# Vasilispapg/CVML-GoalNet

Measured on AMD Instinct MI355X. Metric: training clips/sec at batch 64, 16-frame 224² clips; logit MAE vs CPU ref, higher is better.
Workload: dtype f32; 1 GPU; AVM train step (forward + broadcast-MSE + backward + fused Adam), 64 clips x 16 frames = 1024 frames of 3x224x224 + 30x30 MFCC per GPU; dropout live (device masks), BatchNorm train mode; frames_per_gpu=1024, h=224, w=224, parallelism=dp1, ddp_semantics=local BN + local MSE per rank, gradient mean (standard DDP), params=1286754369

## Files before the change

### cvml_goalnet_amd/csrc/gemm_f32.hip

```cpp
#include <stdlib.h>

#include "gemm_common.h"
#include "skinny.h"

using namespace goalnet;

namespace {

constexpr int BM = 128, BN = 128, BK = 32;
constexpr int LDR = 128;
constexpr int OP_FLOATS = BM * BK;

__device__ __forceinline__ int kc_off(int row, int chunk) { return row * BK + ((chunk ^ ((row >> 1) & 7)) << 2); }

__device__ __forceinline__ float4 f4zero() { return make_float4(0.f, 0.f, 0.f, 0.f); }
__device__ __forceinline__ float4 f4fma(float4 v, float4 s, float4 t) {
    return make_float4(fmaf(v.x, s.x, t.x), fmaf(v.y, s.y, t.y), fmaf(v.z, s.z, t.z), fmaf(v.w, s.w, t.w));
}

typedef unsigned int u32x4 __attribute__((ext_vector_type(4)));
constexpr unsigned OOB = 0xFFFFFF00u;

__device__ __forceinline__ float4 f4sel(bool v, float4 a) { return v ? a : f4zero(); }

// ... 329 lines not shown
    for (int j = blockIdx.x * blockDim.x + threadIdx.x; j < Mpad / 4; j += gridDim.x * blockDim.x) {
        const int kt = j >> 3, k0 = j & 7;
        uint32_t word = 0;
#pragma unroll
        for (int i = 0; i < 4; ++i) {
            const int m = kt * 32 + k0 + 8 * i;
            const int w = m % W, h = (m / W) % H;
            const uint32_t c = m < M ? (uint32_t)((h == 0 ? 1 : 0) | (h == H - 1 ? 2 : 0) | (w == 0 ? 4 : 0) | (w == W - 1 ? 8 : 0)) : 0xFu;
            word |= c << (8 * i);
        }
        codes4[j] = word;
    }
}

__global__ __launch_bounds__(256) void wgrad_border_sums_kernel(const float* __restrict__ dy, double* __restrict__ parts,
                                                               int H, int W, int Cout) {
    const int n = blockIdx.x;
    const float* f = dy + (int64_t)n * H * W * Cout;
    double* out = parts + (int64_t)n * 8 * Cout;
    for (int c = threadIdx.x; c < Cout; c += blockDim.x) {
        double r0 = 0, r1 = 0, c0 = 0, c1 = 0;
        for (int w = 0; w < W; ++w) { r0 += (double)f[(int64_t)w * Cout + c]; r1 += (double)f[((int64_t)(H - 1) * W + w) * Cout + c]; }
        for (int h = 0; h < H; ++h) { c0 += (double)f[(int64_t)h * W * Cout + c]; c1 += (double)f[((int64_t)h * W + W - 1) * Cout + c]; }
        out[0 * Cout + c] = r0; out[1 * Cout + c] = r1; out[2 * Cout + c] = c0; out[3 * Cout + c] = c1;
        out[4 * Cout + c] = (double)f[c];
        out[5 * Cout + c] = (double)f[(int64_t)(W - 1) * Cout + c];
        out[6 * Cout + c] = (double)f[(int64_t)(H - 1) * W * Cout + c];
        out[7 * Cout + c] = (double)f[((int64_t)(H - 1) * W + W - 1) * Cout + c];
    }
}

__device__ __forceinline__ float border_u_of(const double* v, int tap) {
    const int kh = tap / 3, kw = tap - 3 * kh;
    double r = (kh == 0 ? v[0] : 0.0) + (kh == 2 ? v[1] : 0.0) + (kw == 0 ? v[2] : 0.0) + (kw == 2 ? v[3] : 0.0);
    if (kh == 0 && kw == 0) r -= v[4];
    if (kh == 0 && kw == 2) r -= v[5];
    if (kh == 2 && kw == 0) r -= v[6];
    if (kh == 2 && kw == 2) r -= v[7];
    return (float)r;
}

__global__ __launch_bounds__(256) void wgrad_border_u_kernel(const double* __restrict__ parts, int N, int Cout, float* __restrict__ u) {
    __shared__ double s[32][8];
    const int cl = threadIdx.x & 31, j = threadIdx.x >> 5;
    const int c = blockIdx.x * 32 + cl;
    double a0 = 0, a1 = 0, a2 = 0, a3 = 0;
    if (c < Cout) {
        const double* q = parts + (int64_t)j * Cout + c;
        int n = 0;
        for (; n + 3 < N; n += 4) {
            a0 += q[(int64_t)n * 8 * Cout]; a1 += q[(int64_t)(n + 1) * 8 * Cout];
            a2 += q[(int64_t)(n + 2) * 8 * Cout]; a3 += q[(int64_t)(n + 3) * 8 * Cout];
        }
        for (; n < N; ++n) a0 += q[(int64_t)n * 8 * Cout];
    }
    s[cl][j] = (a0 + a1) + (a2 + a3);
    __syncthreads();
    for (int t = threadIdx.x; t < 32 * 9; t += 256) {
        const int cc = t / 9, tap = t - 9 * cc;
        if (blockIdx.x * 32 + cc < Cout) u[(int64_t)(blockIdx.x * 32 + cc) * 9 + tap] = border_u_of(s[cc], tap);
    }
}

template <bool KC>
__device__ __forceinline__ void store_tile(float* l, const float4 (&r)[4], int tid) {
    if (KC) {
        const int c4 = (tid & 7) * 4, row = tid >> 3;
#pragma unroll
        for (int i = 0; i < 4; ++i) *reinterpret_cast<float4*>(&l[kc_off(row + 32 * i, c4 >> 2)]) = r[i];
    } else {
        const int r4 = (tid & 31) * 4, k = tid >> 5;
#pragma unroll
        for (int i = 0; i < 4; ++i) *reinterpret_cast<float4*>(&l[(k + 8 * i) * LDR + r4]) = r[i];
    }
}

template <bool KC>
__device__ __forceinline__ void read_group(const float* l, int strip, int s, int r, int h, float (&f)[2][4]) {
    if (KC) {
#pragma unroll
        for (int q = 0; q < 2; ++q) {
            const float4 t = *reinterpret_cast<const float4*>(&l[kc_off(strip + q * 32 + r, 2 * s + h)]);
            f[q][0] = t.x; f[q][1] = t.y; f[q][2] = t.z; f[q][3] = t.w;
        }
    } else {
#pragma unroll
        for (int j = 0; j < 4; ++j) {
            const float2 t = *reinterpret_cast<const float2*>(&l[(8 * s + 4 * h + j) * LDR + strip + 2 * r]);
            f[0][j] = t.x; f[1][j] = t.y;
        }
    }
}

template <bool AKC, bool BKC>
__device__ __forceinline__ void compute_tile(const float* la, const float* lb, f32x16 (&acc)[2][2],
                                             int wm, int wn, int r, int h) {
#pragma unroll
    for (int s = 0; s < 4; ++s) {
        float a[2][4], b[2][4];
        read_group<AKC>(la, wm * 64, s, r, h, a);
        read_group<BKC>(lb, wn * 64, s, r, h, b);
#pragma unroll
        for (int j = 0; j < 4; ++j) {
#pragma unroll
            for (int fm = 0; fm < 2; ++fm)
#pragma unroll
                for (int fn = 0; fn < 2; ++fn)
                    acc[fm][fn] = __builtin_amdgcn_mfma_f32_32x32x2f32(a[fm][j], b[fn][j], acc[fm][fn], 0, 0, 0);
        }
    }
}

template <bool BKC>
__device__ __forceinline__ void compute_tile_strip(const float* ls, const float* lb, f32x16 (&acc)[2][2],
                                                   const unsigned (&ab)[2], int wn, int r, int h) {
    static_assert(BKC, "K-contiguous B image");
    const unsigned bb = (unsigned)kc_off(wn * 64 + r, h) * 4;
#pragma unroll
    for (int s = 0; s < 4; ++s) {
        float a[2][4], b[2][4];
#pragma unroll
        for (int q = 0; q < 2; ++q) {
            const float4 t = *reinterpret_cast<const float4*>(reinterpret_cast<const char*>(ls) + (ab[q] ^ (unsigned)(s << 5)));
            a[q][0] = t.x; a[q][1] = t.y; a[q][2] = t.z; a[q][3] = t.w;
            const float4 u = *reinterpret_cast<const float4*>(reinterpret_cast<const char*>(lb) + ((bb ^ (unsigned)(s << 5)) + q * 32 * BK * 4));
            b[q][0] = u.x; b[q][1] = u.y; b[q][2] = u.z; b[q][3] = u.w;
        }
#pragma unroll
        for (int j = 0; j < 4; ++j) {
#pragma unroll
            for (int fm = 0; fm < 2; ++fm)
#pragma unroll
                for (int fn = 0; fn < 2; ++fn)
                    acc[fm][fn] = __builtin_amdgcn_mfma_f32_32x32x2f32(a[fm][j], b[fn][j], acc[fm][fn], 0, 0, 0);
        }
    }
}

template <class AL, class BL>
__device__ __forceinline__ void conv_strip_loop(AL& al, BL& bl, float* ls, float* lb, f32x16 (&acc)[2][2], int ktiles,
                                                int tid, int wn, int r, int h) {
    float4 rs[STRIP_LOADS], rb[4];
    const int nchunks = ktiles / 9;
    if (tid < 8) *reinterpret_cast<float4*>(&ls[STRIP_ROWS * BK + tid * 4]) = f4zero();
    al.begin(0);
#pragma unroll
    for (int i = 0; i < STRIP_LOADS; ++i) rs[i] = al.load(0, i);
    bl.issue(0, rb);
    al.store(ls, rs, tid);
    bl.finish(rb);
    store_tile<BL::KC>(lb, rb, tid);
    __syncthreads();
    for (int chunk = 0; chunk < nchunks; ++chunk) {
        const bool next = chunk + 1 < nchunks;
#pragma unroll
        for (int tap = 0; tap < 9; ++tap) {
            const bool more = tap < 8 || next;
            if (more) bl.issue(chunk * 9 + tap + 1, rb);
            if (next) rs[tap] = al.load(chunk + 1, tap);
            unsigned ab[2];
            al.frag_base(tap, ab);
            compute_tile_strip<BL::KC>(ls, lb, acc, ab, wn, r, h);
            __syncthreads();
            if (more) {
                bl.finish(rb);
                store_tile<BL::KC>(lb, rb, tid);
            }
            if (tap == 8 && next) {
                al.begin(chunk + 1);
                al.store(ls, rs, tid);
            }
            __syncthreads();
        }
    }
}

__device__ __forceinline__ void compute_tile_n64(const float* la, const float* lb, f32x16 (&acc)[2], int wave, int r, int h) {
#pragma unroll
    for (int s = 0; s < 4; ++s) {
        const float4 ta = *reinterpret_cast<const float4*>(&la[kc_off(wave * 32 + r, 2 * s + h)]);
        const float4 tb0 = *reinterpret_cast<const float4*>(&lb[kc_off(r, 2 * s + h)]);
        const float4 tb1 = *reinterpret_cast<const float4*>(&lb[kc_off(32 + r, 2 * s + h)]);
        const float a[4] = {ta.x, ta.y, ta.z, ta.w}, b0[4] = {tb0.x, tb0.y, tb0.z, tb0.w}, b1[4] = {tb1.x, tb1.y, tb1.z, tb1.w};
#pragma unroll
        for (int j = 0; j < 4; ++j) {
            acc[0] = __builtin_amdgcn_mfma_f32_32x32x2f32(a[j], b0[j], acc[0], 0, 0, 0);
            acc[1] = __builtin_amdgcn_mfma_f32_32x32x2f32(a[j], b1[j], acc[1], 0, 0, 0);
        }
    }
}

__device__ __forceinline__ void store_acc_n64(const EpiP& ep, const f32x16 (&acc)[2], int tm, int tn, int split, int wave, int r, int h) {
    float* outp = ep.slab_stride > 0 ? (ep.slabs ? ep.slabs : ep.out) + (int64_t)split * ep.slab_stride : ep.out;
    const int mode = ep.slab_stride > 0 ? EPI_RAW : ep.mode;
    const int64_t ld = (ep.slab_stride > 0 && ep.slabs) ? (int64_t)ep.cols : ep.ld;
#pragma unroll
    for (int fn = 0; fn < 2; ++fn) {
        const int col = tn * 64 + fn * 32 + r;
        const bool colok = col < ep.cols;
        const int64_t row0 = (int64_t)tm * BM + wave * 32 + 4 * h;
        const float bv = (mode == EPI_BIAS_RELU && ep.bias) ? ep.bias[colok ? col : 0] : 0.f;
        const float lo = (mode == EPI_BIAS_RELU && ep.relu) ? 0.f : -INFINITY;
#pragma unroll
        for (int e = 0; e < 16; ++e) {
            const int64_t row = row0 + (e & 3) + 8 * (e >> 2);
            if (!(colok && row < ep.rows)) continue;
            const float v = acc[fn][e];
            if (mode == EPI_RAW) outp[row * ld + col] = v;
            else if (mode == EPI_BIAS_RELU) outp[row * ld + col] = fmaxf(v + bv, lo);
            else outp[row * ld + col] = epi_apply(ep, v, row, col);
        }
    }
}

template <class AL, class BL, bool N64 = false, int STAGES = 2>
__global__ __launch_bounds__(256, STAGES == 1 ? (N64 ? 4 : AL::ONE_STAGE_BLOCKS) : 2) void gemm_f32_kernel(typename AL::P ap, typename BL::P bp, EpiP ep,
                                                          int tiles_m, int tiles_n, int m_fast,
                                                          int ktiles, int ktiles_per_split, int xcd_splits) {
    const int tid = threadIdx.x;
    int tm, tn, split;
    if (xcd_splits > 0) {
        const int tiles = tiles_m * tiles_n;
        const int xcd = blockIdx.x & 7, j = blockIdx.x >> 3;
        int t;
        if (tiles > 64 && tiles <= 128) {
            const int gs = (xcd_splits + 7) / 8, rest = tiles - 64, nA = gs * 64;
            int q;
            if (j < nA) { q = j >> 6; t = j & 63; }
            else { const int i = j - nA; q = i / rest; t = 64 + (i - q * rest); }
            split = q * 8 + xcd;
        } else {
            split = (j / tiles) * 8 + xcd;
            t = j - (j / tiles) * tiles;
        }
        if (split >= xcd_splits) return;
        if (m_fast) { tm = t % tiles_m; tn = t / tiles_m; } else { tn = t % tiles_n; tm = t / tiles_n; }
    } else {
        tile_of_block(tiles_m, tiles_n, m_fast, tm, tn);
        split = blockIdx.y;
    }
    const int kt0 = split * ktiles_per_split;
    const int kt1 = min(ktiles, kt0 + ktiles_per_split);

    static_assert(!N64 || (AL::KC && BL::KC), "the 128 x 64 tile reads K-contiguous LDS images");
    AL al(ap, tm * BM, tid);
    BL bl(bp, tn * (N64 ? 64 : BN), tid);

    const int lane = tid & 63, wave = tid >> 6;
    const int wm = wave >> 1, wn = wave & 1;
    const int r = lane & 31, h = lane >> 5;

    f32x16 acc[2][2];
#pragma unroll
    for (int i = 0; i < 2; ++i)
#pragma unroll
        for (int j = 0; j < 2; ++j)
#pragma unroll
            for (int e = 0; e < 16; ++e) acc[i][j][e] = 0.f;

    if constexpr (AL::STRIP) {
        static_assert(!N64 && STAGES == 1 && BL::KC, "the strip form: 128 x 128 tile, one B stage");
        __shared__ __attribute__((aligned(16))) float lstrip[STRIP_FLOATS];
        __shared__ __attribute__((aligned(16))) float lbs[OP_FLOATS];
        conv_strip_loop(al, bl, lstrip, lbs, acc, kt1 - kt0, tid, wn, r, h);
    } else {
        __shared__ __attribute__((aligned(16))) float lds[STAGES][2][OP_FLOATS];
        float4 ra[4], rb[4];
        if (kt0 < kt1) {
            al.issue(kt0, ra);
            bl.issue(kt0, rb);
            al.finish(ra);
            bl.finish(rb);
            store_tile<AL::KC>(lds[0][0], ra, tid);
            store_tile<BL::KC>(lds[0][1], rb, tid);
        }
        __syncthreads();
        for (int kt = kt0; kt < kt1; ++kt) {
            const int cur = STAGES == 1 ? 0 : (kt - kt0) & 1;
            const bool more = kt + 1 < kt1;
            if (more) {
                al.issue(kt + 1, ra);
                bl.issue(kt + 1, rb);
            }
            if constexpr (N64) compute_tile_n64(lds[cur][0], lds[cur][1], acc[0], wave, r, h);
            else compute_tile<AL::KC, BL::KC>(lds[cur][0], lds[cur][1], acc, wm, wn, r, h);
            if constexpr (STAGES == 1) __syncthreads();
            if (more) {
                al.finish(ra);
                bl.finish(rb);
                store_tile<AL::KC>(lds[STAGES == 1 ? 0 : cur ^ 1][0], ra, tid);
                store_tile<BL::KC>(lds[STAGES == 1 ? 0 : cur ^ 1][1], rb, tid);
            }
            __syncthreads();
        }
    }
    if constexpr (N64) store_acc_n64(ep, acc[0], tm, tn, split, wave, r, h);
    else store_acc<!AL::KC, !BL::KC>(ep, acc, tm, tn, split, wm, wn, r, h);
    if (ep.tile_ctr) {
        const int nsp = (ktiles + ktiles_per_split - 1) / ktiles_per_split;
        fused_splitk_reduce<N64 ? 64 : BN>(ep, tm, tn, tm * tiles_n + tn, nsp, tid);
    }
}

__global__ __launch_bounds__(256) void splitk_reduce_kernel(const float* slabs, int nsplit, int64_t slab_stride, EpiP ep) {
    const int c4n = ep.cols >> 2;
    const int64_t total = (int64_t)ep.rows * c4n;
    for (int64_t i = (int64_t)blockIdx.x * blockDim.x + threadIdx.x; i < total; i += (int64_t)gridDim.x * blockDim.x) {
        const int64_t row = i / c4n;
        const int col = (int)(i - row * c4n) * 4;
        const float* s = slabs + row * ep.cols + col;
        float4 a = *reinterpret_cast<const float4*>(s);
        for (int k = 1; k < nsplit; ++k) {
            const float4 b = *reinterpret_cast<const float4*>(s + (int64_t)k * slab_stride);
            a.x += b.x; a.y += b.y; a.z += b.z; a.w += b.w;
        }
        if (ep.oscale) { const int k = *ep.oscale; a.x = ldexpf(a.x, k); a.y = ldexpf(a.y, k); a.z = ldexpf(a.z, k); a.w = ldexpf(a.w, k); }
        if (ep.corr_u) {
            const int tap = col / ep.corr_C, ci = col - tap * ep.corr_C;
            const float u = ep.corr_u[row * 9 + tap];
            const float4 shv = *reinterpret_cast<const float4*>(ep.corr_sh + ci);
            a.x = fmaf(-shv.x, u, a.x); a.y = fmaf(-shv.y, u, a.y); a.z = fmaf(-shv.z, u, a.z); a.w = fmaf(-shv.w, u, a.w);
        }
        float* o = ep.out + row * ep.ld + col;
        o[0] = epi_apply(ep, a.x, row, col);
        o[1] = epi_apply(ep, a.y, row, col + 1);
        o[2] = epi_apply(ep, a.z, row, col + 2);
        o[3] = epi_apply(ep, a.w, row, col + 3);
    }
}

__global__ __launch_bounds__(256) void splitk_reduce_wide_kernel(const float* slabs, int nsplit, int64_t slab_stride, EpiP ep) {
    const int c4n = ep.cols >> 2;
    const int64_t total = (int64_t)ep.rows * c4n;
    const int g = threadIdx.x & 15;
    const int64_t step = (int64_t)gridDim.x * 16;
    const int64_t rounds = (total + step - 1) / step;
    int64_t i = (int64_t)blockIdx.x * 16 + (threadIdx.x >> 4);
    for (int64_t r = 0; r < rounds; ++r, i += step) {
        const bool ok = i < total;
        const int64_t ic = ok ? i : 0;
        const int64_t row = ic / c4n;
        const int col = (int)(ic - row * c4n) * 4;
        const float* s = slabs + row * ep.cols + col;
        float4 a = make_float4(0.f, 0.f, 0.f, 0.f);
        for (int k = g; k < nsplit; k += 16) {
            const float4 b = *reinterpret_cast<const float4*>(s + (int64_t)k * slab_stride);
            a.x += b.x; a.y += b.y; a.z += b.z; a.w += b.w;
        }
        a.x = row16_sum(a.x); a.y = row16_sum(a.y); a.z = row16_sum(a.z); a.w = row16_sum(a.w);
        if (ep.oscale) { const int k = *ep.oscale; a.x = ldexpf(a.x, k); a.y = ldexpf(a.y, k); a.z = ldexpf(a.z, k); a.w = ldexpf(a.w, k); }
        if (ep.corr_u) {
            const int tap = col / ep.corr_C, ci = col - tap * ep.corr_C;
            const float u = ep.corr_u[row * 9 + tap];
            const float4 shv = *reinterpret_cast<const float4*>(ep.corr_sh + ci);
            a.x = fmaf(-shv.x, u, a.x); a.y = fmaf(-shv.y, u, a.y); a.z = fmaf(-shv.z, u, a.z); a.w = fmaf(-shv.w, u, a.w);
        }
        if (ok && g == 0) {
            float* o = ep.out + row * ep.ld + col;
            o[0] = epi_apply(ep, a.x, row, col);
            o[1] = epi_apply(ep, a.y, row, col + 1);
            o[2] = epi_apply(ep, a.z, row, col + 2);
            o[3] = epi_apply(ep, a.w, row, col + 3);
        }
    }
}

template <class AL, class BL, bool N64 = false>
int launch_gemm(const char* name, const typename AL::P& ap, const typename BL::P& bp, const EpiP& ep,
                int64_t M, int64_t N, int ktiles, int nsplit, int m_fast, hipStream_t st) {
    const int64_t tiles_m = (M + BM - 1) / BM, tiles_n = (N + (N64 ? 64 : BN) - 1) / (N64 ? 64 : BN);
    GN_REQUIRE(tiles_m * tiles_n < (1ll << 31), GOALNET_E_SHAPE, "%s: too many tiles", name);
    GN_REQUIRE(nsplit >= 1 && nsplit <= 65535, GOALNET_E_SHAPE, "%s: bad split count %d", name, nsplit);
    const int kps = (ktiles + nsplit - 1) / nsplit;
    GN_REQUIRE(!ep.tile_ctr || (ktiles + kps - 1) / kps == nsplit, GOALNET_E_SHAPE, "%s: fused split-K needs every split non-empty", name);
    const bool xcd_local = nsplit >= 8 && tiles_m * tiles_n <= 256 && tiles_m * tiles_n * ((nsplit + 7) / 8 * 8) < (1ll << 31);
    dim3 grid((unsigned)(tiles_m * tiles_n), (unsigned)nsplit, 1);
    if (xcd_local) grid = dim3((unsigned)(tiles_m * tiles_n * ((nsplit + 7) / 8 * 8)), 1, 1);
    static const int force_stages = getenv("GOALNET_F32_STAGES") ? atoi(getenv("GOALNET_F32_STAGES")) : 0;
    const bool one_stage = AL::STRIP || force_stages == 1 || (force_stages != 2 && AL::ONE_STAGE);
    if (one_stage) {
        hipLaunchKernelGGL((gemm_f32_kernel<AL, BL, N64, 1>), grid, dim3(256), 0, st, ap, bp, ep, (int)tiles_m, (int)tiles_n,
                           m_fast, ktiles, kps, xcd_local ? nsplit : 0);
        GN_LAUNCH_CHECK(name);
        return 0;
    }
    if constexpr (!AL::STRIP) {
        hipLaunchKernelGGL((gemm_f32_kernel<AL, BL, N64>), grid, dim3(256), 0, st, ap, bp, ep, (int)tiles_m, (int)tiles_n,
                           m_fast, ktiles, kps, xcd_local ? nsplit : 0);
        GN_LAUNCH_CHECK(name);
    }
    return 0;
}

}

namespace goalnet {
int launch_splitk_reduce(const char* name, const float* slabs, int nsplit, int64_t slab_stride, const EpiP& ep, hipStream_t st) {
    const int64_t total = (int64_t)ep.rows * (ep.cols >> 2);
    int64_t blocks = (total + 255) / 256;
    if (blocks > 4096) blocks = 4096;
    if (blocks < 1) blocks = 1;
    if (total < 65536 && nsplit >= 32) {
        int64_t wb = (total + 15) / 16;
        if (wb > 4096) wb = 4096;
        hipLaunchKernelGGL(splitk_reduce_wide_kernel, dim3((unsigned)wb), dim3(256), 0, st, slabs, nsplit, slab_stride, ep);
        GN_LAUNCH_CHECK(name);
        return 0;
    }
    hipLaunchKernelGGL(splitk_reduce_kernel, dim3((unsigned)blocks), dim3(256), 0, st, slabs, nsplit, slab_stride, ep);
    GN_LAUNCH_CHECK(name);
    return 0;
}

int pick_splits(int64_t tiles, int ktiles) {
    if (ktiles < 8 || (ktiles < 64 && tiles >= 128)) return 1;
    int64_t s = ((ktiles < 64 ? 256 : 1024) + tiles - 1) / tiles;
    const int64_t smax = ktiles < 64 ? ktiles / 4 : (ktiles / 8 > 1 ? ktiles / 8 : 1);
    if (s > smax) s = smax;
    if (s < 1) s = 1;
    const int kps = (int)((ktiles + s - 1) / s);
    return (ktiles + kps - 1) / kps;
}

}

extern "C" {

static int conv_splits_f32(int64_t M, int Cin, int Cout) {
    return conv_fwd_splits(((M + BM - 1) / BM) * ((Cout + BN - 1) / BN), 9 * Cin / BK);
}

constexpr bool CONV_STRIP_FWD = true;
constexpr bool CONV_STRIP_DGRAD = true;
static bool conv_strip_f32(int W, int nsplit, bool narrow, bool affine) {
    const char* e = getenv("GOALNET_F32_CONV_STRIP");
    if (e && e[0] == '0') return false;
    return nsplit == 1 && !narrow && W <= CONV_STRIP_MAX_W && (affine ? CONV_STRIP_FWD : CONV_STRIP_DGRAD);
}

size_t goalnet_conv3x3_fwd_ws_bytes(int N, int H, int W, int Cin, int Cout) {
    if (N <= 0 || H <= 0 || W <= 0 || Cin <= 0 || Cout <= 0) return 0;
    const int64_t M = (int64_t)N * H * W;
    const int s = conv_splits_f32(M, Cin, Cout);
    return s > 1 ? (size_t)s * (size_t)M * (size_t)Cout * sizeof(float) : 0;
}

int goalnet_conv3x3_fwd(const float* x, const float* scale, const float* shift, const float* w,
                        const float* bias, int relu, float* y, int N, int H, int W, int Cin, int Cout,
                        void* ws, size_t ws_bytes, int* tile_ctr, int n_ctr, void* stream) {
    GN_REQUIRE(x && w && y, GOALNET_E_NULL, "conv3x3_fwd: null pointer");
    GN_REQUIRE((scale == nullptr) == (shift == nullptr), GOALNET_E_NULL, "conv3x3_fwd: scale/shift must both be set or both NULL");
    GN_REQUIRE(N > 0 && H > 0 && W > 0 && Cin > 0 && Cout > 0, GOALNET_E_SHAPE, "conv3x3_fwd: non-positive dim");
    GN_REQUIRE(Cin % BK == 0, GOALNET_E_SHAPE, "conv3x3_fwd: Cin=%d must be a multiple of %d", Cin, BK);
    GN_REQUIRE(Cout % 4 == 0, GOALNET_E_SHAPE, "conv3x3_fwd: Cout=%d must be a multiple of 4", Cout);
    GN_REQUIRE(aligned16(x) && aligned16(w) && aligned16(y) && aligned16(scale) && aligned16(shift),
               GOALNET_E_ALIGN, "conv3x3_fwd: pointers must be 16-byte aligned");
    const int64_t M = (int64_t)N * H * W;
    GN_REQUIRE(M < (1ll << 31) - 256, GOALNET_E_SHAPE, "conv3x3_fwd: N*H*W too large");
    hipStream_t st = (hipStream_t)stream;
    KCLoader<false>::P bp{w, (int64_t)9 * Cin, Cout, nullptr, nullptr, 1, Cin};
    const EpiP efinal{EPI_BIAS_RELU, y, Cout, (int)M, Cout, bias, relu, nullptr, 0, nullptr, 0, 0};
    EpiP ep = efinal;
    const int ktiles = 9 * Cin / BK;
    int nsplit = ws ? conv_splits_f32(M, Cin, Cout) : 1;
    if (nsplit > 1) {
        GN_REQUIRE(aligned16(ws) && ws_bytes >= goalnet_conv3x3_fwd_ws_bytes(N, H, W, Cin, Cout), GOALNET_E_WORKSPACE,
                   "conv3x3_fwd: workspace too small or misaligned");
        ep = EpiP{EPI_RAW, (float*)ws, Cout, (int)M, Cout, nullptr, 0, nullptr, 0, nullptr, 0, M * Cout};
    }
    const bool narrow = Cout <= 64 && !getenv("GOALNET_F32_N64_OFF");
    const bool fused = nsplit > 1 && tile_ctr && (int64_t)n_ctr >= ((M + BM - 1) / BM) * ((Cout + (narrow ? 64 : BN) - 1) / (narrow ? 64 : BN));
    if (fused) {
        ep = efinal;
        ep.slabs = (float*)ws; ep.slab_stride = M * Cout; ep.tile_ctr = tile_ctr;
    }
    const bool strip = conv_strip_f32(W, nsplit, narrow, scale != nullptr);
    int rc;
    if (strip && scale) {
        ConvAStripLoader<true>::P ap{x, H, W, Cin, M, scale, shift};
        rc = launch_gemm<ConvAStripLoader<true>, KCLoader<false>>("conv3x3_fwd", ap, bp, ep, M, Cout, ktiles, 1, 0, st);
    } else if (strip) {
        ConvAStripLoader<false>::P ap{x, H, W, Cin, M, nullptr, nullptr};
        rc = launch_gemm<ConvAStripLoader<false>, KCLoader<false>>("conv3x3_fwd", ap, bp, ep, M, Cout, ktiles, 1, 0, st);
    } else if (scale) {
        ConvALoader<true>::P ap{x, H, W, Cin, M, scale, shift};
        rc = narrow ? launch_gemm<ConvALoader<true>, KCLoader<false>, true>("conv3x3_fwd", ap, bp, ep, M, Cout, ktiles, nsplit, 0, st)
                    : launch_gemm<ConvALoader<true>, KCLoader<false>>("conv3x3_fwd", ap, bp, ep, M, Cout, ktiles, nsplit, 0, st);
    } else {
        ConvALoader<false>::P ap{x, H, W, Cin, M, nullptr, nullptr};
        rc = narrow ? launch_gemm<ConvALoader<false>, KCLoader<false>, true>("conv3x3_fwd", ap, bp, ep, M, Cout, ktiles, nsplit, 0, st)
                    : launch_gemm<ConvALoader<false>, KCLoader<false>>("conv3x3_fwd", ap, bp, ep, M, Cout, ktiles, nsplit, 0, st);
    }
    if (rc || nsplit == 1 || fused) return rc;
    return launch_splitk_reduce("conv3x3_fwd.reduce", (const float*)ws, nsplit, M * Cout, efinal, st);
}

}
namespace {
template <class AL, class BL, bool N64, int STAGES> const char* gemm_f32_kernel_name_() { return __PRETTY_FUNCTION__; }
template <class AL, class BL, bool N64> const char* gemm_f32_kernel_name() {
    const int force = getenv("GOALNET_F32_STAGES") ? atoi(getenv("GOALNET_F32_STAGES")) : 0;
    const bool one = AL::STRIP || force == 1 || (force != 2 && AL::ONE_STAGE);
    return one ? gemm_f32_kernel_name_<AL, BL, N64, 1>() : gemm_f32_kernel_name_<AL, BL, N64, 2>();
}
}
extern "C" {

const char* goalnet_conv3x3_fwd_kernel_name(int N, int H, int W, int Cin, int Cout, int affine) {
    const bool narrow = Cout <= 64 && !getenv("GOALNET_F32_N64_OFF");
    const int nsplit = (N > 0 && H > 0 && W > 0 && Cin > 0 && Cout > 0) ? conv_splits_f32((int64_t)N * H * W, Cin, Cout) : 1;
    if (conv_strip_f32(W, nsplit, narrow, affine != 0))
        return affine ? gemm_f32_kernel_name<ConvAStripLoader<true>, KCLoader<false>, false>()
                      : gemm_f32_kernel_name<ConvAStripLoader<false>, KCLoader<false>, false>();
    if (affine) return narrow ? gemm_f32_kernel_name<ConvALoader<true>, KCLoader<false>, true>() : gemm_f32_kernel_name<ConvALoader<true>, KCLoader<false>, false>();
    return narrow ? gemm_f32_kernel_name<ConvALoader<false>, KCLoader<false>, true>() : gemm_f32_kernel_name<ConvALoader<false>, KCLoader<false>, false>();
}

static int wgrad_splits(int64_t M, int Cin, int Cout) {
    const int64_t tiles = (int64_t)((Cout + BM - 1) / BM) * ((9 * Cin + BN - 1) / BN);
    const int ktiles = (int)((M + BK - 1) / BK);
    static const int wtarget = getenv("GOALNET_WGRAD_SPLIT_TARGET") ? atoi(getenv("GOALNET_WGRAD_SPLIT_TARGET")) : 2048;
    int64_t s = (wtarget + tiles - 1) / tiles;
    const int64_t smax = ktiles / 4 > 1 ? ktiles / 4 : 1;
    if (s > smax) s = smax;
    if (s > 512) s = 512;
    if (s >= 8) {
        int64_t best = (s + 7) / 8 * 8 <= smax ? (s + 7) / 8 * 8 : s / 8 * 8;
        double best_eff = 0.0;
        for (int64_t c = best; c <= 2 * s + 8 && c <= smax && c <= 1024; c += 8) {
            const int64_t blocks = tiles * c, rounds = (blocks + 511) / 512;
            const double eff = (double)blocks / (double)(rounds * 512);
            if (eff > best_eff + 1e-9) { best_eff = eff; best = c; }
        }
        s = best;
    }
    const int kps = (int)((ktiles + s - 1) / s);
    return (ktiles + kps - 1) / kps;
}

static size_t wgrad_codes_bytes(int64_t M) { return (size_t)((M + 31) / 32 * 32 + 255) / 256 * 256; }
static size_t wgrad_border_bytes(int N, int Cout) {
    return ((size_t)N * 8 * Cout * sizeof(double) + 255) / 256 * 256 + ((size_t)Cout * 9 * sizeof(float) + 255) / 256 * 256;
}

size_t goalnet_conv3x3_wgrad_ws_bytes(int N, int H, int W, int Cin, int Cout) {
    const int64_t M = (int64_t)N * H * W;
    return wgrad_codes_bytes(M) + wgrad_border_bytes(N, Cout) + (size_t)wgrad_splits(M, Cin, Cout) * (size_t)Cout * 9 * Cin * sizeof(float);
}

int goalnet_conv3x3_wgrad_codes(uint32_t* codes, int N, int H, int W, void* stream) {
    GN_REQUIRE(codes && N > 0 && H > 0 && W > 0, GOALNET_E_NULL, "conv3x3_wgrad_codes: bad arguments");
    const int64_t M = (int64_t)N * H * W;
    GN_REQUIRE(M < (1ll << 31) - 256, GOALNET_E_SHAPE, "conv3x3_wgrad_codes: N*H*W too large");
    const int Mpad = (int)((M + 31) / 32 * 32);
    int blocks = (Mpad / 4 + 255) / 256;
    if (blocks > 4096) blocks = 4096;
    hipLaunchKernelGGL(border_codes_kernel, dim3(blocks), dim3(256), 0, (hipStream_t)stream, codes, (int)M, Mpad, H, W);
    GN_LAUNCH_CHECK("conv3x3_wgrad_codes");
    return 0;
}

size_t goalnet_conv3x3_wgrad_codes_bytes(int N, int H, int W) { return wgrad_codes_bytes((int64_t)N * H * W); }

int goalnet_conv3x3_wgrad(const float* x, const float* scale, const float* shift, const float* dy, float* dw,
                          void* ws, size_t ws_bytes, const uint32_t* codes_in, int* tile_ctr, int n_ctr,
                          int N, int H, int W, int Cin, int Cout, void* stream) {
    GN_REQUIRE(x && dy && dw && ws, GOALNET_E_NULL, "conv3x3_wgrad: null pointer");
    GN_REQUIRE((scale == nullptr) == (shift == nullptr), GOALNET_E_NULL, "conv3x3_wgrad: scale/shift must both be set or both NULL");
    GN_REQUIRE(N > 0 && H > 0 && W > 0, GOALNET_E_SHAPE, "conv3x3_wgrad: non-positive dim");
    GN_REQUIRE(Cin % 4 == 0 && Cout % 4 == 0 && Cin > 0 && Cout > 0, GOALNET_E_SHAPE, "conv3x3_wgrad: channels must be multiples of 4");
    GN_REQUIRE(aligned16(x) && aligned16(dy) && aligned16(dw) && aligned16(ws) && aligned16(scale) && aligned16(shift),
               GOALNET_E_ALIGN, "conv3x3_wgrad: pointers must be 16-byte aligned");
    const int64_t M = (int64_t)N * H * W;
    GN_REQUIRE(M < (1ll << 31) - 256, GOALNET_E_SHAPE, "conv3x3_wgrad: N*H*W too large");
    GN_REQUIRE(ws_bytes >= goalnet_conv3x3_wgrad_ws_bytes(N, H, W, Cin, Cout), GOALNET_E_WORKSPACE, "conv3x3_wgrad: workspace too small");
    hipStream_t st = (hipStream_t)stream;
    const int nsplit = wgrad_splits(M, Cin, Cout);
    const int ktiles = (int)((M + BK - 1) / BK);
    const int64_t slab = (int64_t)Cout * 9 * Cin;
    uint32_t* codes = (uint32_t*)ws;
    double* bparts = (double*)((char*)ws + wgrad_codes_bytes(M));
    float* bu = (float*)((char*)bparts + ((size_t)N * 8 * Cout * sizeof(double) + 255) / 256 * 256);
    float* slabs = (float*)((char*)ws + wgrad_codes_bytes(M) + wgrad_border_bytes(N, Cout));
    const char* force = getenv("GOALNET_WGRAD_PATH");
    const bool dsel = force && force[0] == 's' ? true : force && force[0] == 'c' ? false : (int64_t)N * (H > W ? H : W) <= 4096;
    if (codes_in) {
        codes = const_cast<uint32_t*>(codes_in);
    } else {
        const int Mpad = (int)((M + 31) / 32 * 32);
        int blocks = (Mpad / 4 + 255) / 256;
        if (blocks > 4096) blocks = 4096;
        hipLaunchKernelGGL(border_codes_kernel, dim3(blocks), dim3(256), 0, st, codes, (int)M, Mpad, H, W);
        GN_LAUNCH_CHECK("conv3x3_wgrad.codes");
    }
    if (scale && !dsel) {
        hipLaunchKernelGGL(wgrad_border_sums_kernel, dim3(N), dim3(256), 0, st, dy, bparts, H, W, Cout);
        GN_LAUNCH_CHECK("conv3x3_wgrad.border_sums");
        hipLaunchKernelGGL(wgrad_border_u_kernel, dim3((Cout + 31) / 32), dim3(256), 0, st, bparts, N, Cout, bu);
        GN_LAUNCH_CHECK("conv3x3_wgrad.border_u");
    }
    MCLoader<false>::P ap{dy, Cout, Cout, (int)M, nullptr, nullptr, 1};
    EpiP ep{EPI_RAW, slabs, (int64_t)9 * Cin, Cout, 9 * Cin, nullptr, 0, nullptr, 0, nullptr, 0, slab};
    const bool fused = nsplit > 1 && tile_ctr && (dsel || !scale) &&
                       (int64_t)n_ctr >= (int64_t)((Cout + BM - 1) / BM) * ((9 * Cin + BN - 1) / BN);
    if (fused) {
        ep = EpiP{EPI_RAW, dw, (int64_t)9 * Cin, Cout, 9 * Cin, nullptr, 0, nullptr, 0, nullptr, 0, slab};
        ep.slabs = slabs; ep.tile_ctr = tile_ctr;
    }
    int rc;
    if (scale && dsel) {
        ConvWgradBLoader<true, true>::P bp{x, H, W, Cin, (int)M, scale, shift, codes};
        rc = launch_gemm<MCLoader<false>, ConvWgradBLoader<true, true>>("conv3x3_wgrad", ap, bp, ep, Cout, 9 * Cin, ktiles, nsplit, 1, st);
    } else if (scale) {
        ConvWgradBLoader<true>::P bp{x, H, W, Cin, (int)M, scale, shift, codes};
        rc = launch_gemm<MCLoader<false>, ConvWgradBLoader<true>>("conv3x3_wgrad", ap, bp, ep, Cout, 9 * Cin, ktiles, nsplit, 1, st);
    } else {
        ConvWgradBLoader<false>::P bp{x, H, W, Cin, (int)M, nullptr, nullptr, codes};
        rc = launch_gemm<MCLoader<false>, ConvWgradBLoader<false>>("conv3x3_wgrad", ap, bp, ep, Cout, 9 * Cin, ktiles, nsplit, 1, st);
    }
    if (rc || fused) return rc;
    EpiP er{EPI_RAW, dw, (int64_t)9 * Cin, Cout, 9 * Cin, nullptr, 0, nullptr, 0, nullptr, 0, 0};
    if (scale && !dsel) { er.corr_u = bu; er.corr_sh = shift; er.corr_C = Cin; }
    return launch_splitk_reduce("conv3x3_wgrad.reduce", slabs, nsplit, slab, er, st);
}

static int linear_splits(int M, int64_t K, int J) {
    const int64_t tiles = (int64_t)((M + BM - 1) / BM) * ((J + BN - 1) / BN);
    return pick_splits(tiles, (int)(K / BK));
}

size_t goalnet_linear_fwd_ws_bytes(int M, int64_t K, int J) {
    if (M <= 0 || K <= 0 || J <= 0) return 0;
    if (M <= SKINNY_MAX_M) return skinny_fwd_ws_bytes(M, K, J);
    const int s = linear_splits(M, K, J);
    return s > 1 ? (size_t)s * (size_t)M * (size_t)J * sizeof(float) : 0;
}

int goalnet_linear_fwd(const float* x, int64_t ldx, const float* scale, const float* shift, int bnC,
                       const float* w, const float* bias, int relu, const float* dropmask, int64_t ldmask,
                       float* y, int64_t ldy, float* mult_out, int64_t ldmult,
                       int M, int64_t K, int J, void* ws, size_t ws_bytes, void* stream) {
    GN_REQUIRE(x && w && y, GOALNET_E_NULL, "linear_fwd: null pointer");
    GN_REQUIRE((scale == nullptr) == (shift == nullptr), GOALNET_E_NULL, "linear_fwd: scale/shift must both be set or both NULL");
    GN_REQUIRE(M > 0 && J > 0 && K > 0 && K < (1ll << 31) - 64, GOALNET_E_SHAPE, "linear_fwd: bad dims");
    GN_REQUIRE(K % BK == 0, GOALNET_E_SHAPE, "linear_fwd: K=%lld must be a multiple of %d", (long long)K, BK);
    GN_REQUIRE(J % 4 == 0, GOALNET_E_SHAPE, "linear_fwd: J=%d must be a multiple of 4", J);
    GN_REQUIRE(!scale || (bnC > 0 && bnC % 4 == 0), GOALNET_E_SHAPE, "linear_fwd: bnC must be a positive multiple of 4");
    GN_REQUIRE(aligned16(x) && aligned16(w) && aligned16(y) && aligned16(scale) && aligned16(shift) && ldx % 4 == 0 && ldy % 4 == 0,
               GOALNET_E_ALIGN, "linear_fwd: pointers / leading dims must be 16-byte aligned");
    hipStream_t st = (hipStream_t)stream;
    EpiP efinal{(dropmask || mult_out) ? EPI_FULL : EPI_BIAS_RELU, y, ldy, M, J, bias, relu, dropmask, ldmask, mult_out, ldmult, 0};
    if (M <= SKINNY_MAX_M) {
        const size_t need = skinny_fwd_ws_bytes(M, K, J);
        GN_REQUIRE(need == 0 || (ws && aligned16(ws) && ws_bytes >= need), GOALNET_E_WORKSPACE, "linear_fwd: workspace too small");
        return skinny_linear_fwd(x, ldx, scale, shift, bnC, w, efinal, M, K, J, ws, st);
    }
    const int nsplit = linear_splits(M, K, J);
    const int ktiles = (int)(K / BK);
    KCLoader<false>::P bp{w, K, J, nullptr, nullptr, 1, 0};
    EpiP ep = efinal;
    if (nsplit > 1) {
        GN_REQUIRE(ws && aligned16(ws), GOALNET_E_WORKSPACE, "linear_fwd: split-K needs a 16-byte aligned workspace");
        GN_REQUIRE(ws_bytes >= goalnet_linear_fwd_ws_bytes(M, K, J), GOALNET_E_WORKSPACE, "linear_fwd: workspace too small");
        ep = EpiP{EPI_RAW, (float*)ws, J, M, J, nullptr, 0, nullptr, 0, nullptr, 0, (int64_t)M * J};
    }
    int rc;
    if (scale) {
        KCLoader<true>::P ap{x, ldx, M, scale, shift, bnC, 0};
        rc = launch_gemm<KCLoader<true>, KCLoader<false>>("linear_fwd", ap, bp, ep, M, J, ktiles, nsplit, 0, st);
    } else {
        KCLoader<false>::P ap{x, ldx, M, nullptr, nullptr, 1, 0};
        rc = launch_gemm<KCLoader<false>, KCLoader<false>>("linear_fwd", ap, bp, ep, M, J, ktiles, nsplit, 0, st);
    }
    if (rc || nsplit == 1) return rc;
    return launch_splitk_reduce("linear_fwd.reduce", (const float*)ws, nsplit, (int64_t)M * J, efinal, st);
}

int goalnet_linear_bwd_dx(const float* dy, int64_t lddy, const float* w, const float* mult, int64_t ldmult,
                          float* dx, int64_t lddx, int M, int64_t K, int J, void* stream) {
    GN_REQUIRE(dy && w && dx, GOALNET_E_NULL, "linear_bwd_dx: null pointer");
    GN_REQUIRE(M > 0 && J > 0 && K > 0 && K < (1ll << 31) - 256, GOALNET_E_SHAPE, "linear_bwd_dx: bad dims");
    GN_REQUIRE(J % BK == 0, GOALNET_E_SHAPE, "linear_bwd_dx: J=%d must be a multiple of %d", J, BK);
    GN_REQUIRE(K % 4 == 0, GOALNET_E_SHAPE, "linear_bwd_dx: K must be a multiple of 4");
    GN_REQUIRE(aligned16(dy) && aligned16(w) && aligned16(dx) && lddy % 4 == 0 && lddx % 4 == 0,
               GOALNET_E_ALIGN, "linear_bwd_dx: pointers / leading dims must be 16-byte aligned");
    hipStream_t st = (hipStream_t)stream;
    if (M <= SKINNY_MAX_M && (!mult || (aligned16(mult) && ldmult % 4 == 0)))
        return skinny_linear_dx(dy, lddy, w, mult, ldmult, dx, lddx, M, K, J, st);
    KCLoader<false>::P ap{dy, lddy, M, nullptr, nullptr, 1, 0};
    MCLoader<false>::P bp{w, K, (int)K, J, nullptr, nullptr, 1};
    EpiP ep{mult ? EPI_MUL : EPI_RAW, dx, lddx, M, (int)K, nullptr, 0, mult, ldmult, nullptr, 0, 0};
    return launch_gemm<KCLoader<false>, MCLoader<false>>("linear_bwd_dx", ap, bp, ep, M, K, J / BK, 1, 1, st);
}

int goalnet_linear_bwd_dw(const float* dy, int64_t lddy, const float* x, int64_t ldx,
                          const float* scale, const float* shift, int bnC,
                          float* dw, float* db, int M, int64_t K, int J, void* stream) {
    GN_REQUIRE(dy && x && dw, GOALNET_E_NULL, "linear_bwd_dw: null pointer");
    GN_REQUIRE((scale == nullptr) == (shift == nullptr), GOALNET_E_NULL, "linear_bwd_dw: scale/shift must both be set or both NULL");
    GN_REQUIRE(M > 0 && J > 0 && K > 0 && K < (1ll << 31) - 256, GOALNET_E_SHAPE, "linear_bwd_dw: bad dims");
    GN_REQUIRE(J % 4 == 0 && K % 4 == 0, GOALNET_E_SHAPE, "linear_bwd_dw: J and K must be multiples of 4");
    GN_REQUIRE(!scale || (bnC > 0 && bnC % 4 == 0), GOALNET_E_SHAPE, "linear_bwd_dw: bnC must be a positive multiple of 4");
    GN_REQUIRE(aligned16(dy) && aligned16(x) && aligned16(dw) && aligned16(scale) && aligned16(shift) && lddy % 4 == 0 && ldx % 4 == 0,
               GOALNET_E_ALIGN, "linear_bwd_dw: pointers / leading dims must be 16-byte aligned");
    hipStream_t st = (hipStream_t)stream;
    if (M <= SKINNY_MAX_M) return skinny_linear_dw(dy, lddy, x, ldx, scale, shift, bnC, dw, db, M, K, J, st);
    if (db) { const int rc = goalnet_colsum(dy, lddy, M, J, db, stream); if (rc) return rc; }
    const int ktiles = (M + BK - 1) / BK;
    MCLoader<false>::P ap{dy, lddy, J, M, nullptr, nullptr, 1};
    EpiP ep{EPI_RAW, dw, K, J, (int)K, nullptr, 0, nullptr, 0, nullptr, 0, 0};
    if (scale) {
        MCLoader<true>::P bp{x, ldx, (int)K, M, scale, shift, bnC};
        return launch_gemm<MCLoader<false>, MCLoader<true>>("linear_bwd_dw", ap, bp, ep, J, K, ktiles, 1, 1, st);
    }
    MCLoader<false>::P bp{x, ldx, (int)K, M, nullptr, nullptr, 1};
    return launch_gemm<MCLoader<false>, MCLoader<false>>("linear_bwd_dw", ap, bp, ep, J, K, ktiles, 1, 1, st);
}

}
```

Measured before the change: 158.2 clips/s.

## Add 128x192 wgrad GEMM tile for conv3x3 weight-gradient layers

Adds a dedicated conv3x3 weight-gradient kernel with a 128x192 output tile (2x3 MFMA 32x32 fragments per wave). It has its own loaders and a single-stage LDS pipeline, and writes raw split-K slabs. It is enabled by default for the Cin=256/Cout=512 and Cin=64/Cout=256 layers when the non-fused, non-dsel path is taken. The wider tile is meant to cut A-operand reloads and tile count for 9*Cin columns that divide by 192. In exchange it raises register pressure (launch bounds 256,3), runs without double buffering, and cannot use the fused split-K reduce.

```diff
diff --git a/cvml_goalnet_amd/csrc/gemm_f32.hip b/cvml_goalnet_amd/csrc/gemm_f32.hip
--- a/cvml_goalnet_amd/csrc/gemm_f32.hip
+++ b/cvml_goalnet_amd/csrc/gemm_f32.hip
@@ -655,6 +655,215 @@
     }
 }
 
+constexpr int BN192 = 192;
+constexpr int OPB192_FLOATS = BK * BN192;
+
+struct WgradALoader192 {
+    using P = MCLoader<false>::P;
+    const float* x;
+    int64_t ld;
+    int kred;
+    unsigned voff0;
+    __device__ WgradALoader192(const P& p, int col0, int tid) {
+        const int col = col0 + (tid & 31) * 4;
+        x = p.x; ld = p.ld; kred = p.kred;
+        voff0 = col < p.cols ? (unsigned)(((int64_t)(tid >> 5) * p.ld + col) * 4) : 0x80000000u;
+    }
+    __device__ __forceinline__ void issue(int kt, float4 (&r)[4]) const {
+        const int kbase = kt * BK;
+        const int nk = kred - kbase < BK ? kred - kbase : BK;
+        const __amdgpu_buffer_rsrc_t rx = make_rsrc(x + (int64_t)kbase * ld, (uint32_t)nk * (uint32_t)ld * 4u);
+        const unsigned step = (unsigned)(8 * ld * 4);
+        unsigned b = voff0;
+        asm volatile("" : "+v"(b));
+#pragma unroll
+        for (int i = 0; i < 4; ++i) r[i] = bload(rx, b + (unsigned)i * step, 0);
+    }
+};
+
+constexpr unsigned WG192_DEAD = 1u << 27;
+constexpr int64_t WG192_MAX_SPAN = 1ll << 26;
+
+template <bool AFFINE>
+struct ConvWgradBLoader192 {
+    using P = typename ConvWgradBLoader<AFFINE>::P;
+    const float* x;
+    __amdgpu_buffer_rsrc_t rcodes;
+    int W, C, M, k0, i1;
+    unsigned vbase[2], bad4[2], nextcode;
+    __device__ ConvWgradBLoader192(const P& p, int col0, int tid, float* coef) {
+        x = p.x; W = p.W; C = p.C; M = p.M; k0 = tid >> 5; i1 = (tid >> 3) & 2;
+        rcodes = make_rsrc(p.codes4, (uint32_t)((p.M + 31) / 32 * 32));
+        nextcode = 0;
+#pragma unroll
+        for (int g = 0; g < 2; ++g) {
+            const int col = col0 + (g == 0 ? (tid & 31) * 4 : 128 + (tid & 15) * 4);
+            const bool dead = col >= 9 * p.C;
+            const int cc = dead ? 0 : col;
+            const int tap = cc / p.C, ci = cc - tap * p.C;
+            const int kh = tap / 3, kw = tap - 3 * kh;
+            bad4[g] = ((kh == 0 ? 1u : 0u) | (kh == 2 ? 2u : 0u) | (kw == 0 ? 4u : 0u) | (kw == 2 ? 8u : 0u)) * 0x01010101u;
+            vbase[g] = dead ? WG192_DEAD : (unsigned)(((k0 + (g == 0 ? 0 : 8 * i1) + kh * p.W + kw) * p.C + ci) * 4);
+        }
+        if (AFFINE && tid < BN192) {
+            const int col = col0 + tid;
+            const int ci = (col < 9 * p.C ? col : 0) % p.C;
+            coef[tid] = p.scale[ci];
+            coef[BN192 + tid] = p.shift[ci];
+        }
+    }
+    __device__ __forceinline__ unsigned load_code(int kt) const {
+        return (unsigned)__builtin_amdgcn_raw_buffer_load_b32(rcodes, k0 * 4, kt * 32, 0);
+    }
+    __device__ __forceinline__ void prime(int kt) { nextcode = load_code(kt); }
+    __device__ __forceinline__ void issue(int kt, float4 (&r)[6]) {
+        const int mbase = kt * BK;
+        const unsigned code = nextcode;
+        const unsigned bad0 = code & bad4[0], bad1 = (code & bad4[1]) >> (8 * i1);
+        const int lead = mbase - (W + 1), lead0 = lead < 0 ? 0 : lead;
+        const int last = mbase + BK + (W + 1) < M ? mbase + BK + (W + 1) : M;
+        const __amdgpu_buffer_rsrc_t rx = make_rsrc(x + (int64_t)lead0 * C, (uint32_t)(last - lead0) * (uint32_t)C * 4u);
+        const unsigned adj = (unsigned)((lead - lead0) * C * 4);
+        const unsigned step = (unsigned)(8 * C * 4);
+        unsigned b0 = vbase[0], b1 = vbase[1];
+        asm volatile("" : "+v"(b0), "+v"(b1));
+        b0 += adj; b1 += adj;
+#pragma unroll
+        for (int i = 0; i < 4; ++i) r[i] = bload(rx, (((bad0 >> (8 * i)) & 0xFu) << 28) + (b0 + (unsigned)i * step), 0);
+#pragma unroll
+        for (int i = 0; i < 2; ++i) r[4 + i] = bload(rx, (((bad1 >> (8 * i)) & 0xFu) << 28) + (b1 + (unsigned)i * step), 0);
+        nextcode = load_code(kt + 1);
+    }
+    __device__ __forceinline__ void finish(float4 (&r)[6], const float* coef, int tid) const {
+        if (AFFINE) {
+            const int c0 = (tid & 31) * 4, c1 = 128 + (tid & 15) * 4;
+            const float4 sc0 = *reinterpret_cast<const float4*>(&coef[c0]), sh0 = *reinterpret_cast<const float4*>(&coef[BN192 + c0]);
+            const float4 sc1 = *reinterpret_cast<const float4*>(&coef[c1]), sh1 = *reinterpret_cast<const float4*>(&coef[BN192 + c1]);
+#pragma unroll
+            for (int i = 0; i < 4; ++i) r[i] = f4fma(r[i], sc0, sh0);
+#pragma unroll
+            for (int i = 0; i < 2; ++i) r[4 + i] = f4fma(r[4 + i], sc1, sh1);
+        }
+    }
+    __device__ __forceinline__ void store(float* l, const float4 (&r)[6], int tid) const {
+#pragma unroll
+        for (int i = 0; i < 4; ++i) *reinterpret_cast<float4*>(&l[(k0 + 8 * i) * BN192 + (tid & 31) * 4]) = r[i];
+#pragma unroll
+        for (int i = 0; i < 2; ++i) *reinterpret_cast<float4*>(&l[(k0 + 8 * (i1 + i)) * BN192 + 128 + (tid & 15) * 4]) = r[4 + i];
+    }
+};
+
+__device__ __forceinline__ void compute_tile192(const float* la, const float* lb, f32x16 (&acc)[2][3], int wm, int wn, int r, int h) {
+    const float* pa = &la[4 * h * LDR + wm * 64 + 2 * r];
+    const float* pb = &lb[4 * h * BN192 + wn * 96 + 2 * r];
+    const float* pc = &lb[4 * h * BN192 + wn * 96 + 64 + r];
+    float2 ta = *reinterpret_cast<const float2*>(pa), tb = *reinterpret_cast<const float2*>(pb);
+    float tc = *pc;
+#pragma unroll
+    for (int t = 0; t < 16; ++t) {
+        const float a0 = ta.x, a1 = ta.y, b0 = tb.x, b1 = tb.y, b2 = tc;
+        if (t < 15) {
+            const int k = 8 * ((t + 1) >> 2) + ((t + 1) & 3);
+            ta = *reinterpret_cast<const float2*>(pa + k * LDR);
+            tb = *reinterpret_cast<const float2*>(pb + k * BN192);
+            tc = pc[k * BN192];
+        }
+        acc[0][0] = __builtin_amdgcn_mfma_f32_32x32x2f32(a0, b0, acc[0][0], 0, 0, 0);
+        acc[0][1] = __builtin_amdgcn_mfma_f32_32x32x2f32(a0, b1, acc[0][1], 0, 0, 0);
+        acc[0][2] = __builtin_amdgcn_mfma_f32_32x32x2f32(a0, b2, acc[0][2], 0, 0, 0);
+        acc[1][0] = __builtin_amdgcn_mfma_f32_32x32x2f32(a1, b0, acc[1][0], 0, 0, 0);
+        acc[1][1] = __builtin_amdgcn_mfma_f32_32x32x2f32(a1, b1, acc[1][1], 0, 0, 0);
+        acc[1][2] = __builtin_amdgcn_mfma_f32_32x32x2f32(a1, b2, acc[1][2], 0, 0, 0);
+        if (t < 15) __builtin_amdgcn_sched_group_barrier(0x100, 3, 0);
+        __builtin_amdgcn_sched_group_barrier(0x008, 6, 0);
+        __builtin_amdgcn_sched_barrier(0);
+    }
+}
+
+__device__ __forceinline__ void store_acc_raw192(const EpiP& ep, const f32x16 (&acc)[2][3], int tm, int tn, int split,
+                                                 int wm, int wn, int r, int h) {
+    float* outp = ep.out + (int64_t)split * ep.slab_stride;
+#pragma unroll
+    for (int fm = 0; fm < 2; ++fm)
+#pragma unroll
+        for (int fn = 0; fn < 3; ++fn) {
+            const int col = tn * BN192 + wn * 96 + (fn < 2 ? 2 * r + fn : 64 + r);
+            const bool colok = col < ep.cols;
+            const int64_t row0 = (int64_t)tm * BM + wm * 64 + fm + 8 * h;
+#pragma unroll
+            for (int e = 0; e < 16; ++e) {
+                const int64_t row = row0 + 2 * ((e & 3) + 8 * (e >> 2));
+                if (colok && row < ep.rows) outp[row * ep.ld + col] = acc[fm][fn][e];
+            }
+        }
+}
+
+template <bool AFFINE>
+__global__ __launch_bounds__(256, 3) void gemm_f32_wgrad192_kernel(MCLoader<false>::P ap, typename ConvWgradBLoader192<AFFINE>::P bp, EpiP ep,
+                                                                   int tiles_m, int tiles_n, int ktiles, int ktiles_per_split, int xcd_splits) {
+    const int tid = threadIdx.x;
+    int tm, tn, split;
+    if (xcd_splits > 0) {
+        const int tiles = tiles_m * tiles_n;
+        const int xcd = blockIdx.x & 7, j = blockIdx.x >> 3;
+        split = (j / tiles) * 8 + xcd;
+        const int t = j - (j / tiles) * tiles;
+        if (split >= xcd_splits) return;
+        tm = t % tiles_m; tn = t / tiles_m;
+    } else {
+        tile_of_block(tiles_m, tiles_n, 1, tm, tn);
+        split = blockIdx.y;
+    }
+    const int kt0 = split * ktiles_per_split;
+    const int kt1 = min(ktiles, kt0 + ktiles_per_split);
+
+    __shared__ __attribute__((aligned(16))) float la[OP_FLOATS];
+    __shared__ __attribute__((aligned(16))) float lb[OPB192_FLOATS];
+    __shared__ __attribute__((aligned(16))) float coef[2 * BN192];
+    WgradALoader192 al(ap, tm * BM, tid);
+    ConvWgradBLoader192<AFFINE> bl(bp, tn * BN192, tid, coef);
+    if (AFFINE) __syncthreads();
+
+    const int lane = tid & 63, wave = tid >> 6;
+    const int wm = wave >> 1, wn = wave & 1;
+    const int r = lane & 31, h = lane >> 5;
+
+    f32x16 acc[2][3];
+#pragma unroll
+    for (int i = 0; i < 2; ++i)
+#pragma unroll
+        for (int j = 0; j < 3; ++j)
+#pragma unroll
+            for (int e = 0; e < 16; ++e) acc[i][j][e] = 0.f;
+
+    float4 ra[4], rb[6];
+    if (kt0 < kt1) {
+        bl.prime(kt0);
+        bl.issue(kt0, rb);
+        al.issue(kt0, ra);
+        bl.finish(rb, coef, tid);
+        store_tile<false>(la, ra, tid);
+        bl.store(lb, rb, tid);
+    }
+    __syncthreads();
+    for (int kt = kt0; kt < kt1; ++kt) {
+        const bool more = kt + 1 < kt1;
+        if (more) {
+            bl.issue(kt + 1, rb);
+            al.issue(kt + 1, ra);
+        }
+        compute_tile192(la, lb, acc, wm, wn, r, h);
+        __syncthreads();
+        if (more) {
+            bl.finish(rb, coef, tid);
+            store_tile<false>(la, ra, tid);
+            bl.store(lb, rb, tid);
+        }
+        __syncthreads();
+    }
+    store_acc_raw192(ep, acc, tm, tn, split, wm, wn, r, h);
+}
+
 __global__ __launch_bounds__(256) void splitk_reduce_kernel(const float* slabs, int nsplit, int64_t slab_stride, EpiP ep) {
     const int c4n = ep.cols >> 2;
     const int64_t total = (int64_t)ep.rows * c4n;
@@ -742,6 +951,28 @@
                            m_fast, ktiles, kps, xcd_local ? nsplit : 0);
         GN_LAUNCH_CHECK(name);
     }
+    return 0;
+}
+
+inline bool wgrad192_spans_ok(int W, int Cin, int64_t Cout) {
+    return (int64_t)(2 * (int64_t)W + 34) * Cin * 4 < WG192_MAX_SPAN && Cout * BK * 4 < WG192_MAX_SPAN;
+}
+
+template <bool AFFINE>
+int launch_wgrad192(const char* name, const MCLoader<false>::P& ap, const typename ConvWgradBLoader192<AFFINE>::P& bp, const EpiP& ep,
+                    int64_t M, int64_t N, int ktiles, int nsplit, hipStream_t st) {
+    const int64_t tiles_m = (M + BM - 1) / BM, tiles_n = (N + BN192 - 1) / BN192;
+    GN_REQUIRE(tiles_m * tiles_n < (1ll << 31), GOALNET_E_SHAPE, "%s: too many tiles", name);
+    GN_REQUIRE(nsplit >= 1 && nsplit <= 65535, GOALNET_E_SHAPE, "%s: bad split count %d", name, nsplit);
+    GN_REQUIRE(ep.slab_stride > 0 && !ep.slabs && !ep.tile_ctr, GOALNET_E_SHAPE, "%s: the 192-wide tile stores raw slabs only", name);
+    GN_REQUIRE(wgrad192_spans_ok(bp.W, bp.C, ap.ld), GOALNET_E_SHAPE, "%s: a K-tile spans too many bytes for the 192-wide tile", name);
+    const int kps = (ktiles + nsplit - 1) / nsplit;
+    const bool xcd_local = nsplit >= 8 && tiles_m * tiles_n <= 256 && tiles_m * tiles_n * ((nsplit + 7) / 8 * 8) < (1ll << 31);
+    dim3 grid((unsigned)(tiles_m * tiles_n), (unsigned)nsplit, 1);
+    if (xcd_local) grid = dim3((unsigned)(tiles_m * tiles_n * ((nsplit + 7) / 8 * 8)), 1, 1);
+    hipLaunchKernelGGL((gemm_f32_wgrad192_kernel<AFFINE>), grid, dim3(256), 0, st, ap, bp, ep, (int)tiles_m, (int)tiles_n,
+                       ktiles, kps, xcd_local ? nsplit : 0);
+    GN_LAUNCH_CHECK(name);
     return 0;
 }
 
@@ -889,6 +1120,18 @@
     }
     const int kps = (int)((ktiles + s - 1) / s);
     return (ktiles + kps - 1) / kps;
+}
+
+constexpr bool WGRAD192_CONV3 = true;
+constexpr bool WGRAD192_CONV2 = true;
+static bool wgrad_tile192_f32(int W, int Cin, int Cout, bool dsel, bool fused) {
+    if (dsel || fused || !wgrad192_spans_ok(W, Cin, Cout)) return false;
+    const char* s = getenv("GOALNET_F32_STAGES");
+    if (s && atoi(s) == 2) return false;
+    const char* e = getenv("GOALNET_F32_WGRAD_TILE");
+    if (e && atoi(e) == 192) return true;
+    if (e && atoi(e) == 128) return false;
+    return (Cin == 256 && Cout == 512 && WGRAD192_CONV3) || (Cin == 64 && Cout == 256 && WGRAD192_CONV2);
 }
 
 static size_t wgrad_codes_bytes(int64_t M) { return (size_t)((M + 31) / 32 * 32 + 255) / 256 * 256; }
@@ -961,7 +1204,15 @@
         ep.slabs = slabs; ep.tile_ctr = tile_ctr;
     }
     int rc;
-    if (scale && dsel) {
+    if (wgrad_tile192_f32(W, Cin, Cout, dsel, fused)) {
+        if (scale) {
+            ConvWgradBLoader192<true>::P bp{x, H, W, Cin, (int)M, scale, shift, codes};
+            rc = launch_wgrad192<true>("conv3x3_wgrad", ap, bp, ep, Cout, 9 * Cin, ktiles, nsplit, st);
+        } else {
+            ConvWgradBLoader192<false>::P bp{x, H, W, Cin, (int)M, nullptr, nullptr, codes};
+            rc = launch_wgrad192<false>("conv3x3_wgrad", ap, bp, ep, Cout, 9 * Cin, ktiles, nsplit, st);
+        }
+    } else if (scale && dsel) {
         ConvWgradBLoader<true, true>::P bp{x, H, W, Cin, (int)M, scale, shift, codes};
         rc = launch_gemm<MCLoader<false>, ConvWgradBLoader<true, true>>("conv3x3_wgrad", ap, bp, ep, Cout, 9 * Cin, ktiles, nsplit, 1, st);
     } else if (scale) {
```

After: 158.7 clips/s, median of 6. No clear change (+0.3%).
